# dwkim606/optimal_conv

Measured on AMD Instinct MI355X. Metric: homomorphic convs/sec (conv_then_pack + BN bias, k x k, batch B, N=2^16), higher is better.
Workload: dtype u64; 1 GPU; conv 3 3; ker_wid=3, batch=256, in_wid=16, logN=16, moduli=ckks.DefaultBootstrapParams[6] Q0,Q1 + P=0x1fffffffffe00001, ciphertexts_per_launch_set=4, contexts_per_gpu=4, chunk_nodes=512

## Files before the change

### optimal_conv_amd/csrc/hc_kernels.h

```cpp
#pragma once
#include "hc_arith.h"

#define HC_TPB 256
#ifndef HC_MIN_WAVES
#define HC_MIN_WAVES 4
#endif
#define HC_ROWS_LDS 4096
#define HC_COLS_LDS 4096

struct __attribute__((aligned(16))) HcTw { u64 w, ws; };

#define HC_SMALL_Q(q) ((q) < (1ull << 31))
template <bool B> struct HcBool { static constexpr bool value = B; };
template <int V> struct HcInt { static constexpr int value = V; };
#define HC_COUNT_DISPATCH(n, body) do { switch (n) { case 1: body(HcInt<1>{}); break; case 2: body(HcInt<2>{}); break; case 3: body(HcInt<3>{}); break; case 4: body(HcInt<4>{}); break; \
    case 5: body(HcInt<5>{}); break; case 6: body(HcInt<6>{}); break; case 7: body(HcInt<7>{}); break; case 8: body(HcInt<8>{}); break; default: break; } } while (0)
#define HC_LD(S32, rowptr, j) ((S32) ? hc_ld32(rowptr, j) : (rowptr)[j])
#define HC_ST(S32, rowptr, j, v) do { if (S32) hc_st32(rowptr, j, v); else (rowptr)[j] = (v); } while (0)
#define HC_ROW_DISPATCH(row32, body) do { if (row32) body(HcBool<true>{}); else body(HcBool<false>{}); } while (0)
__device__ __forceinline__ u64 hc_ld32(const u64 *row, size_t j) { return (u64)reinterpret_cast<const u32 *>(row)[j]; }
__device__ __forceinline__ void hc_st32(u64 *row, size_t j, u64 v) { reinterpret_cast<u32 *>(row)[j] = (u32)v; }
struct __attribute__((packed, aligned(4))) HcU64A4 { u64 v; };
__device__ __forceinline__ u64 hc_ldp(const u64 *row, size_t j, bool row32) {
    return reinterpret_cast<const HcU64A4 *>(reinterpret_cast<const char *>(row) + (j << (row32 ? 2 : 3)))->v & (row32 ? 0xFFFFFFFFull : ~0ull);
// ... 146 lines not shown
    hc_gs_round<false>(e, HcRowsTwA<KC>{T.rowsA + row * 16}, Q, T.ninv, T.ninv);
}
template <int FM, bool KC = false>
__device__ __forceinline__ void hc_cols_fwd(u64 (&e)[16], u64 *lds, const HcTwTab &T, int c, int tid, const HcQ &Q) {
    hc_ct_round<FM>(e, HcRowsTwA<KC>{T.colsA}, Q);
#pragma unroll
    for (int hi = 0; hi < 16; hi++) lds[hc_cols_lds(hi * 16 + tid, c)] = e[hi];
    __syncthreads();
#pragma unroll
    for (int lo = 0; lo < 16; lo++) e[lo] = lds[hc_cols_lds(tid * 16 + lo, c)];
    hc_ct_round<FM>(e, HcRowsTwB<KC>{T.colsB + tid}, Q);
}
template <bool SCALE = true, bool KC = false>
__device__ __forceinline__ void hc_cols_inv(u64 (&e)[16], u64 *lds, const HcTwTab &T, int c, int tid, const HcQ &Q) {
    hc_gs_round<false>(e, HcRowsTwB<KC>{T.colsB + tid}, Q, T.ninv, T.ninv);
#pragma unroll
    for (int lo = 0; lo < 16; lo++) lds[hc_cols_lds(tid * 16 + lo, c)] = e[lo];
    __syncthreads();
#pragma unroll
    for (int hi = 0; hi < 16; hi++) e[hi] = lds[hc_cols_lds(hi * 16 + tid, c)];
    hc_gs_round<SCALE>(e, HcRowsTwA<KC>{T.colsA}, Q, T.ninv, T.w_last_ninv);
}

__device__ __forceinline__ void hc_rows_inv_f64(double (&e)[16], u64 *lds, const HcTwTab &T, int row, int rloc, int tid, HcF64Mod m) {
    hc_gs_round_f64<false>(e, HcRowsTwB<false>{T.rowsB + row * 256 + tid}, m, T.ninv, T.ninv);
#pragma unroll
    for (int lo = 0; lo < 16; lo++) lds[hc_rows_lds(rloc, tid * 16 + lo)] = hc_d2u(e[lo]);
    HC_ROW_SYNC();
#pragma unroll
    for (int hi = 0; hi < 16; hi++) e[hi] = hc_u2d(lds[hc_rows_lds(rloc, hi * 16 + tid)]);
    hc_gs_round_f64<false>(e, HcRowsTwA<false>{T.rowsA + row * 16}, m, T.ninv, T.ninv);
}
__device__ __forceinline__ void hc_cols_inv_f64(double (&e)[16], u64 *lds, const HcTwTab &T, int c, int tid, HcF64Mod m) {
    hc_gs_round_f64<false>(e, HcRowsTwB<false>{T.colsB + tid}, m, T.ninv, T.ninv);
#pragma unroll
    for (int lo = 0; lo < 16; lo++) lds[hc_cols_lds(tid * 16 + lo, c)] = hc_d2u(e[lo]);
    __syncthreads();
#pragma unroll
    for (int hi = 0; hi < 16; hi++) e[hi] = hc_u2d(lds[hc_cols_lds(hi * 16 + tid, c)]);
    hc_gs_round_f64<true>(e, HcRowsTwA<false>{T.colsA}, m, T.ninv, T.w_last_ninv);
}

__device__ __forceinline__ void hc_rows_lin_to_lo(u64 (&e)[16], u64 *lds, int t, int rloc, int tid) {
#pragma unroll
    for (int k = 0; k < 16; k++) lds[hc_rows_lds(k, t)] = e[k];
    __syncthreads();
#pragma unroll
    for (int lo = 0; lo < 16; lo++) e[lo] = lds[hc_rows_lds(rloc, tid * 16 + lo)];
}
__device__ __forceinline__ void hc_rows_lo_to_lin(u64 (&e)[16], u64 *lds, int t, int rloc, int tid) {
#pragma unroll
    for (int lo = 0; lo < 16; lo++) lds[hc_rows_lds(rloc, tid * 16 + lo)] = e[lo];
    __syncthreads();
#pragma unroll
    for (int k = 0; k < 16; k++) e[k] = lds[hc_rows_lds(k, t)];
// ... 443 lines not shown
__global__ __launch_bounds__(HC_TPB) void hc_k_permute_mm(const u64 *in, u64 *out, u32 g, size_t is, const HcMod *mods, int nl, int nq, int nt) {
    const size_t base = (size_t)blockIdx.z * is + (size_t)blockIdx.y * 65536;
    const int T = (int)blockIdx.y % nt; const bool row32 = mods[T < nl ? T : nq + (T - nl)].row32 != 0;
    auto body = [&](auto s32c) {
    constexpr bool S32 = decltype(s32c)::value;
    for (size_t i = (size_t)blockIdx.x * HC_TPB + threadIdx.x; i < 65536; i += (size_t)gridDim.x * HC_TPB) HC_ST(S32, out + base, i, HC_LD(S32, in + base, hc_perm_src((u32)i, g)));
    };
    HC_ROW_DISPATCH(row32, body);
}

__global__ __launch_bounds__(HC_TPB) void hc_k_rotate_finish(const u64 *d0, const u64 *d1, const u64 *c0, u64 *o0, u64 *o1, const HcMod *mods, u32 g, size_t is) {
    const int l = blockIdx.y; const u64 q = mods[l].q; const size_t base = (size_t)l * 65536 + (size_t)(blockIdx.z >> 1) * is;
    auto body = [&](auto s32c) {
    constexpr bool S32 = decltype(s32c)::value;
    if ((blockIdx.z & 1) == 0) {
        for (size_t i = (size_t)blockIdx.x * HC_TPB + threadIdx.x; i < 65536; i += (size_t)gridDim.x * HC_TPB) { const size_t s = hc_perm_src((u32)i, g); HC_ST(S32, o0 + base, i, hc_addmod(HC_LD(S32, d0 + base, s), HC_LD(S32, c0 + base, s), q)); }
    } else {
        for (size_t i = (size_t)blockIdx.x * HC_TPB + threadIdx.x; i < 65536; i += (size_t)gridDim.x * HC_TPB) HC_ST(S32, o1 + base, i, HC_LD(S32, d1 + base, hc_perm_src((u32)i, g)));
    }
    };
    HC_ROW_DISPATCH(mods[l].row32, body);
}

#ifndef HC_JOB_FAST
#define HC_JOB_FAST 0
#endif
#if HC_JOB_FAST
#define HC_JOB blockIdx.x
#define HC_TILE blockIdx.y
#define HC_NJOBS gridDim.x
#else
#define HC_JOB blockIdx.y
#define HC_TILE blockIdx.x
#define HC_NJOBS gridDim.y
#endif
#define HC_FREE_OFF 72
#ifndef HC_W_A1
#define HC_W_A1 4
#endif
#ifndef HC_W_A2
#define HC_W_A2 4
#endif
#ifndef HC_W_A3
#define HC_W_A3 4
#endif
#ifndef HC_W_B1
#define HC_W_B1 4
#endif
#ifndef HC_W_B2
#define HC_W_B2 1
#endif
#ifndef HC_W_B3
#define HC_W_B3 4
#endif
#ifndef HC_W_B4
#define HC_W_B4 1
#endif
struct HcLoopA {
    const HcTw *ctc;
    HcPtrs ker;
    u64 *tmp;
    u64 *cts;
    int i0, norm;
    int slot0, slot_step;
    size_t cts_stride;
    int njobs;
    HcMod m0, m1;
    HcTw q1inv;
    u64 h, negh0;
};
#ifndef HC_A_WAVES
#define HC_A_WAVES 4
#endif
template <int F64>
__global__ __launch_bounds__(HC_TPB, HC_W_A1) void hc_k_a1(HcLoopA A, HcTwTab T1inv) {
    __shared__ hc_cvr_lds_t lds[HC_ROWS_LDS];
    const int t = threadIdx.x, tid = t & 15, rloc = t >> 4, row = HC_TILE * 16 + rloc;
    const int job = HC_JOB, p = job & 1, i = A.i0 + (job >> 1) * A.norm, z = blockIdx.z;
    const HcTw *__restrict__ c = A.ctc + ((size_t)z * 4 + (size_t)p * 2 + 1) * 65536;
    const u64 *__restrict__ k = A.ker.p[z] + ((size_t)i * 2 + 1) * 65536;
    const HcQ Q = hc_q(A.m1.q);
    u64 e[16];
#pragma unroll
    for (int kk = 0; kk < 16; kk++) {
        const size_t off = (size_t)(HC_TILE * 16 + kk) * 256 + t;
        const HcTw cw = c[off];
        e[kk] = hc_shoup4(k[off], cw.w, cw.ws, Q);
    }
    u64 *o = A.tmp + ((size_t)z * A.njobs + job) * 65536 + (size_t)row * 256;
    hc_rows_lin_to_lo(e, lds, t, rloc, tid);
    HC_ROW_SYNC();
    if (F64) {
        const HcF64Mod m{(double)A.m1.q, 1.0 / (double)A.m1.q};
        double f[16];
#pragma unroll
        for (int kk = 0; kk < 16; kk++) f[kk] = hc_f64_reduce(hc_f64_from_u(e[kk]), m.q, m.qinv);
        hc_rows_inv_f64(f, lds, T1inv, row, rloc, tid, m);
#pragma unroll
        for (int hi = 0; hi < 16; hi++) o[hi * 16 + tid] = hc_d2u(f[hi]);
    } else {
        hc_rows_inv(e, lds, T1inv, row, rloc, tid, Q);
#pragma unroll
        for (int hi = 0; hi < 16; hi++) o[hi * 16 + tid] = e[hi];
    }
}
template <int FM, int F64>
__global__ __launch_bounds__(HC_TPB, HC_W_A2) void hc_k_a2(HcLoopA A, HcTwTab T1inv, HcTwTab T0fwd) {
    __shared__ hc_cvc_lds_t lds[HC_COLS_LDS];
    const int t = threadIdx.x, c = t & 15, tid = t >> 4;
    u64 *base = A.tmp + (size_t)HC_JOB * 65536 + HC_TILE * 16 + c;
    const HcQ Q0 = hc_q(A.m0.q);
    u64 e[16];
#pragma unroll
    for (int lo = 0; lo < 16; lo++) e[lo] = base[(size_t)(tid * 16 + lo) * 256];
    if (F64) {
        const double q1 = (double)A.m1.q, hh = (double)A.h;
        const HcF64Mod m{q1, 1.0 / q1};
        double f[16];
#pragma unroll
        for (int lo = 0; lo < 16; lo++) f[lo] = hc_u2d(e[lo]);
        hc_cols_inv_f64(f, lds, T1inv, c, tid, m);
#pragma unroll
        for (int hi = 0; hi < 16; hi++) {
            double v = f[hi];
            v = v > hh ? v - q1 : (v < -hh ? v + q1 : v);
            e[hi] = hc_f64_to_u_plus(v, A.m0.q);
        }
    } else {
        const HcQ Q1 = hc_q(A.m1.q);
        hc_cols_inv(e, lds, T1inv, c, tid, Q1);
#pragma unroll
        for (int hi = 0; hi < 16; hi++) {
            const u64 v = hc_csub(hc_canon4(e[hi], Q1) + A.h, A.m1.q);
            e[hi] = hc_reduce64(v + A.negh0, A.m0.mu, Q0);
        }
    }
    __syncthreads();
    hc_cols_fwd<FM>(e, lds, T0fwd, c, tid, Q0);
#pragma unroll
    for (int lo = 0; lo < 16; lo++) base[(size_t)(tid * 16 + lo) * 256] = e[lo];
}
template <int FM>
__global__ __launch_bounds__(HC_TPB, HC_W_A3) void hc_k_a3(HcLoopA A, HcTwTab T0fwd) {
    __shared__ hc_cvr_lds_t lds[HC_ROWS_LDS];
    const int t = threadIdx.x, tid = t & 15, rloc = t >> 4, row = HC_TILE * 16 + rloc;
    const int job = HC_JOB, p = job & 1, i = A.i0 + (job >> 1) * A.norm, z = blockIdx.z;
    const u64 *__restrict__ in = A.tmp + ((size_t)z * A.njobs + job) * 65536 + (size_t)row * 256;
    const HcTw *__restrict__ c = A.ctc + ((size_t)z * 4 + (size_t)p * 2) * 65536 + (size_t)HC_TILE * 4096 + t;
    const u64 *__restrict__ k = A.ker.p[z] + ((size_t)i * 2) * 65536 + (size_t)HC_TILE * 4096 + t;
    u64 *__restrict__ o = A.cts + (size_t)z * A.cts_stride + ((size_t)(A.slot0 + (job >> 1) * A.slot_step) * 2 + p) * 65536 + (size_t)HC_TILE * 4096 + t;
    const HcQ Q = hc_q(A.m0.q);
    u64 e[16], a0[16];
#pragma unroll
    for (int hi = 0; hi < 16; hi++) e[hi] = in[hi * 16 + tid];
#pragma unroll
    for (int kk = 0; kk < 16; kk++) a0[kk] = k[kk * 256];
#pragma unroll
    for (int kk = 0; kk < 16; kk++) { const HcTw cw = c[kk * 256]; a0[kk] = hc_shoup4(a0[kk], cw.w, cw.ws, Q); }
    hc_rows_fwd<FM>(e, lds, T0fwd, row, rloc, tid, Q);
    HC_ROW_SYNC();
    hc_rows_lo_to_lin(e, lds, t, rloc, tid);
#pragma unroll
    for (int kk = 0; kk < 16; kk++) {
        const u64 d = FM == HC_FM_FREE ? a0[kk] + HC_FREE_OFF * Q.q - e[kk] : a0[kk] + Q.q - hc_canon8(e[kk], Q);
        o[kk * 256] = hc_canon4(hc_shoup4(d, A.q1inv.w, A.q1inv.ws, Q), Q);
    }
}

struct HcLoopB {
    const u64 *src;
    u64 *dst;
    u64 *tmpC;
    u64 *tmpE;
    u64 *tmpT;
    const HcTw *idx;
    const HcTw *evkQ;
    const HcTw *evkP;
    const u64 *idxM;
    const u64 *evkQM;
    int n0, step, norm;
    int nodes;
    size_t src_stride, dst_stride;
    HcMod m0, mp;
    HcTw pmodq;
    HcTw pinv;
    u64 mu0;
    u64 vthresh;
    u32 gal;
// ... 25 lines not shown
    hc_rows_inv(e, lds, T0inv, row, rloc, tid, Q);
    u64 *__restrict__ o = B.tmpC + (size_t)job * 65536 + (size_t)row * 256;
#pragma unroll
    for (int hi = 0; hi < 16; hi++) o[hi * 16 + tid] = e[hi];
}
template <int FMP>
__global__ __launch_bounds__(HC_TPB, HC_W_B2) void hc_k_b2(HcLoopB B, HcTwTab T0inv, HcTwTab TPfwd) {
    __shared__ hc_cvc_lds_t lds[HC_COLS_LDS];
    const int t = threadIdx.x, c = t & 15, tid = t >> 4;
    u64 *base = B.tmpC + (size_t)HC_JOB * 65536 + HC_TILE * 16 + c;
    const HcQ Q0 = hc_q(B.m0.q), QP = hc_q(B.mp.q);
    u64 e[16];
#pragma unroll
    for (int lo = 0; lo < 16; lo++) e[lo] = base[(size_t)(tid * 16 + lo) * 256];
    hc_cols_inv(e, lds, T0inv, c, tid, Q0);
#pragma unroll
    for (int hi = 0; hi < 16; hi++) e[hi] = hc_canon4(e[hi], Q0);
    __syncthreads();
    hc_cols_fwd<FMP>(e, lds, TPfwd, c, tid, QP);
#pragma unroll
    for (int lo = 0; lo < 16; lo++) base[(size_t)(tid * 16 + lo) * 256] = e[lo];
}
template <int FMP>
__global__ __launch_bounds__(HC_TPB, HC_W_B3) void hc_k_b3(HcLoopB B, HcTwTab TPfwd, HcTwTab TPinv) {
    __shared__ hc_cvr_lds_t lds[HC_ROWS_LDS];
    const int t = threadIdx.x, tid = t & 15, rloc = t >> 4, row = HC_TILE * 16 + rloc;
    const int node = HC_JOB;
    const u64 *in = B.tmpC + (size_t)node * 65536 + (size_t)row * 256;
    const HcQ Q = hc_q(B.mp.q);
    u64 cp[16], e[16];
#pragma unroll
    for (int hi = 0; hi < 16; hi++) cp[hi] = in[hi * 16 + tid];
    hc_rows_fwd<FMP>(cp, lds, TPfwd, row, rloc, tid, Q);
#pragma unroll
    for (int k = 0; k < 2; k++) {
        const HcTw *__restrict__ ev = B.evkP + (size_t)k * 65536 + (size_t)HC_TILE * 4096 + t;
#pragma unroll
        for (int lo = 0; lo < 16; lo++) {
            const HcTw w = ev[lo * 256];
            e[lo] = hc_shoup4(cp[lo], w.w, w.ws, Q);
        }
        HC_ROW_SYNC();
        hc_rows_inv(e, lds, TPinv, row, rloc, tid, Q);
        u64 *o = B.tmpE + ((size_t)node * 2 + k) * 65536 + (size_t)row * 256;
#pragma unroll
        for (int hi = 0; hi < 16; hi++) o[hi * 16 + tid] = e[hi];
    }
}
template <int FM>
__global__ __launch_bounds__(HC_TPB, HC_W_B4) void hc_k_b4(HcLoopB B, HcTwTab TPinv, HcTwTab T0fwd) {
    __shared__ hc_cvc_lds_t lds[HC_COLS_LDS];
    const int t = threadIdx.x, c = t & 15, tid = t >> 4;
    u64 *base = B.tmpE + (size_t)HC_JOB * 65536 + HC_TILE * 16 + c;
    const HcQ QP = hc_q(B.mp.q), Q = hc_q(B.m0.q);
    u64 e[16];
#pragma unroll
    for (int lo = 0; lo < 16; lo++) e[lo] = base[(size_t)(tid * 16 + lo) * 256];
    hc_cols_inv<false>(e, lds, TPinv, c, tid, QP);
#pragma unroll
    for (int hi = 0; hi < 16; hi++) {
        const u64 yv = hc_canon4(e[hi], QP);
        u64 r = hc_shoup4(yv, B.pinv.w, B.pinv.ws, Q);
        if (yv >= B.vthresh) r += Q.q - 1;
        e[hi] = r;
    }
    __syncthreads();
    hc_cols_fwd<FM>(e, lds, T0fwd, c, tid, Q);
#pragma unroll
    for (int lo = 0; lo < 16; lo++) base[(size_t)(tid * 16 + lo) * 256] = e[lo];
}
// ... 52 lines not shown
                u64 f;
                if (k == 0) hc_b5_terms<FM, 1>(Y[j], T[j], K[j], X[j], I[j], Q, t1[kk], f);
                else hc_b5_terms<FM, 0>(Y[j], T[j], K[j], X[j], I[j], Q, t1[kk], f);
                if (bias != nullptr) t1[kk] = FM == HC_FM_FREE ? t1[kk] + bias[kk * 256] : hc_addmod(t1[kk], bias[kk * 256], q);
                lds[hc_rows_lds(kk, t)] = FM == HC_FM_FREE ? f + HC_FREE_OFF * q - e[kk] : hc_submod(f, hc_canon8(e[kk], Q), q);
            }
        }
        __syncthreads();
#pragma unroll
        for (int kk = 0; kk < 16; kk++) {
            const u32 srcidx = hc_perm_src((u32)((HC_TILE * 16 + kk) * 256 + t), B.gal);
            const u64 d = lds[hc_rows_lds((int)((srcidx >> 8) & 15), (int)(srcidx & 255))];
            o[kk * 256] = FM == HC_FM_FREE ? hc_reduce64(t1[kk] + d, B.m0.mu, Q) : hc_addmod(t1[kk], d, q);
        }
    }
}

#ifndef HC_B5_ROWS
#define HC_B5_ROWS 4
#endif
#ifndef HC_B5M_WAVES
#define HC_B5M_WAVES 2
#endif
template <int FM, class TW>
__device__ __forceinline__ void hc_ct_round2(u64 (&e0)[16], u64 (&e1)[16], const TW &tw, const HcQ &Q) {
#pragma unroll
    for (int s = 0; s < 4; s++) {
        const int half = 8 >> s;
#pragma unroll
        for (int g = 0; g < (1 << s); g++) {
            const HcTw w = tw((1 << s) - 1 + g);
#pragma unroll
            for (int k = 0; k < half; k++) {
                const int a = g * 2 * half + k, b = a + half;
                u64 X0 = e0[a], X1 = e1[a];
                if (FM == HC_FM_ALT) { X0 = hc_fold(X0, Q.nq4); X1 = hc_fold(X1, Q.nq4); }
                const u64 T0 = hc_shoup4(e0[b], w.w, w.ws, Q), T1 = hc_shoup4(e1[b], w.w, w.ws, Q);
                e0[a] = X0 + T0; e0[b] = (X0 + Q.q4) - T0;
                e1[a] = X1 + T1; e1[b] = (X1 + Q.q4) - T1;
            }
        }
    }
}
template <int FM>
__device__ __forceinline__ void hc_rows_fwd2_lin(u64 (&e0)[16], u64 (&e1)[16], u64 *l0, u64 *l1, const HcTwTab &T, int row, int rloc, int tid, int t, const HcQ &Q) {
    hc_ct_round2<FM>(e0, e1, HcRowsTwA<false>{T.rowsA + row * 16}, Q);
#pragma unroll
    for (int hi = 0; hi < 16; hi++) { const int a = hc_rows_lds(rloc, hi * 16 + tid); l0[a] = e0[hi]; l1[a] = e1[hi]; }
    HC_ROW_SYNC();
#pragma unroll
    for (int lo = 0; lo < 16; lo++) { const int a = hc_rows_lds(rloc, tid * 16 + lo); e0[lo] = l0[a]; e1[lo] = l1[a]; }
    hc_ct_round2<FM>(e0, e1, HcRowsTwB<false>{T.rowsB + row * 256 + tid}, Q);
    HC_ROW_SYNC();
#pragma unroll
    for (int lo = 0; lo < 16; lo++) { const int a = hc_rows_lds(rloc, tid * 16 + lo); l0[a] = e0[lo]; l1[a] = e1[lo]; }
    __syncthreads();
#pragma unroll
    for (int k = 0; k < 16; k++) { const int a = hc_rows_lds(k, t); e0[k] = l0[a]; e1[k] = l1[a]; }
}
template <int FM>
__global__ __launch_bounds__(HC_TPB, HC_B5M_WAVES) void hc_k_b5m(HcLoopB B, HcTwTab T0fwd, HcPtrs biases, HcPtrs outs) {
    __shared__ u64 lds[2 * HC_ROWS_LDS];
    u64 *l0 = lds, *l1 = lds + HC_ROWS_LDS;
    const int t = threadIdx.x, tid = t & 15, rloc = t >> 4, row = HC_TILE * 16 + rloc;
    const int zn = HC_JOB, z = zn / B.nodes, node = zn - z * B.nodes, i = (B.n0 + node) * B.norm;
    const HcQ Q = hc_q(B.m0.q);
// ... 1436 lines not shown
```

### optimal_conv_amd/csrc/hconv.hip

```cpp
#ifdef HC_EMU
#include "hip_emu.h"
#else
#include <hip/hip_runtime.h>
#endif

#include <math.h>
#include <stdarg.h>
#include <stdio.h>
#include <string.h>

#include <map>
#include <utility>
#include <string>
#include <vector>

#include "../../include/hconv.h"
#include "../../include/hconv_test_hooks.h"
#include "hc_kernels.h"
#include "hc_gomath.h"
#ifndef HC_GX_LV
#define HC_GX_LV 64
#endif
#ifndef HC_GX_PW
#define HC_GX_PW 32
// ... 667 lines not shown
    c->ws_ctc = nullptr; c->ws_ctc_cts = 0;
    HC_HIP(c, hcx_malloc(c, (void **)&c->ws_ctc, nct * 4 * HC_N * sizeof(HcTw)));
    c->ws_ctc_cts = nct;
    return HC_OK;
}
static int hc_prepare_ctc(hc_ctx *c, const HcPtrs &ct_in, int n, const u64 cst[2]) {
    HC_TRY(hc_ensure_ctc(c, (size_t)n));
    HcCtc K; K.m0 = c->mods[0].m; K.m1 = c->mods[1].m;
    K.c0 = h_pair(cst[0] % K.m0.q, K.m0.q); K.c1 = h_pair(cst[1] % K.m1.q, K.m1.q);
    return hc_launch(c, "ctc", hc_k_ctc_pairs, dim3(64, 4, (unsigned)n), ct_in, c->ws_ctc, K);
}

static int hc_loopA_run_set(hc_ctx *c, const HcPtrs &kers, int n, int i_first, int i_stride, int nch, u64 *cts, size_t cts_stride, bool compact) {
    long chunk = (c->chunk_nodes < 1 ? 1 : c->chunk_nodes) / n; if (chunk < 1) chunk = 1;
    if (chunk > nch) chunk = nch;
    HC_TRY(hc_ensure_tmp(c, (size_t)n * (size_t)chunk * 2));
    HcLoopA A; HC_TRY(hc_fill_loopA(c, &A, kers, cts, cts_stride, i_stride));
    const HcModHost &m0 = c->mods[0], &m1 = c->mods[1];
    for (int j0 = 0; j0 < nch; j0 += (int)chunk) {
        const int nj = (int)((nch - j0) < chunk ? (nch - j0) : chunk);
        A.i0 = i_first + j0 * i_stride;
        A.slot0 = compact ? j0 : A.i0; A.slot_step = compact ? 1 : i_stride;
        A.njobs = 2 * nj;
        const dim3 grid = hc_grid(2 * nj, n), flat = hc_grid(2 * nj * n);
        if (hc_f64_ok(m1.m.q)) {
            HC_TRY(hc_launch(c, "a1_mul_rowsinv", hc_k_a1<1>, grid, A, m1.inv_f64));
            HC_TRY(hc_fm_free(m0.m.q) ? hc_launch(c, "a2_colsinv_lift_colsfwd", hc_k_a2<HC_FM_FREE, 1>, flat, A, m1.inv_f64, m0.fwd)
                                      : hc_launch(c, "a2_colsinv_lift_colsfwd", hc_k_a2<HC_FM_ALT, 1>, flat, A, m1.inv_f64, m0.fwd));
        } else {
            HC_TRY(hc_launch(c, "a1_mul_rowsinv", hc_k_a1<0>, grid, A, m1.inv));
            HC_TRY(hc_fm_free(m0.m.q) ? hc_launch(c, "a2_colsinv_lift_colsfwd", hc_k_a2<HC_FM_FREE, 0>, flat, A, m1.inv, m0.fwd)
                                      : hc_launch(c, "a2_colsinv_lift_colsfwd", hc_k_a2<HC_FM_ALT, 0>, flat, A, m1.inv, m0.fwd));
        }
        HC_TRY(HC_LAUNCH_FM(m0.m.q, c, "a3_rowsfwd_rescale", hc_k_a3, grid, A, m0.fwd));
    }
    return HC_OK;
}
static int hc_loopA_run(hc_ctx *c, const u64 *ker, int max_ob, int norm, u64 *cts) {
    return hc_loopA_run_set(c, hc_ptrs1(ker), 1, 0, norm, max_ob / norm, cts, 0, false);
}

static int hc_rescale_plan(hc_ctx *c, int level, const HcTw **out) {
    auto it = c->rescale_plan.find(level);
    if (it == c->rescale_plan.end()) {
        const u64 qL = c->mods[(size_t)level].m.q;
        std::vector<HcTw> h((size_t)level);
        for (int i = 0; i < level; i++) { const u64 q = c->mods[(size_t)i].m.q; h[(size_t)i] = h_pair(h_inv(qL % q, q), q); }
        HcTw *d = nullptr; HC_HIP(c, hcx_malloc(c, (void **)&d, h.size() * sizeof(HcTw)));
        HC_HIP(c, hcx_h2d(c, d, h.data(), h.size() * sizeof(HcTw)));
        it = c->rescale_plan.emplace(level, d).first;
    }
    *out = it->second;
    return HC_OK;
}
static int hc_div_round_last_n(hc_ctx *c, int level, const u64 *x, size_t xs, u64 *out, size_t os, int np) {
    if (level < 1 || level >= c->nq) return hc_fail(c, HC_ERR_ARG, "hc_div_round_last: level %d outside 1..%d", level, c->nq - 1);
    if (!x || !out) return hc_fail(c, HC_ERR_ARG, "hc_div_round_last: null");
// ... 227 lines not shown
    HC_TRY(hc_ensure_tmp(c, (size_t)n * chunk * 4));
    HcLoopB B; HC_TRY(hc_fill_loopB(c, &B, src, dst, it->second, logStep, step, norm, galEl, n * chunk));
    B.src_stride = sstride; B.dst_stride = dstride;
    if (it->second.row256) B.tmpT = nullptr;
    HcPtrs nobias; memset(&nobias, 0, sizeof nobias);
    const HcModHost &m0 = c->mods[0], &mp = c->mods[(size_t)c->nq];
    for (int n0 = 0; n0 < nodes; n0 += chunk) {
        const int nn = (nodes - n0) < chunk ? (nodes - n0) : chunk;
        B.n0 = n0; B.nodes = nn;
        const dim3 g1 = hc_grid(n * nn), g2 = hc_grid(2 * n * nn);
        if (c->small_levels > 0 && (long)n * nn <= c->small_levels && it->second.row256 && !HC_JOB_FAST) {
            const HcPtrs pb = bias_last ? *bias_last : nobias, po = outs_last ? *outs_last : nobias;
            B.tmpT = nullptr;
            const dim3 s1(HC_STILES, (unsigned)(n * nn)), s2(HC_STILES, (unsigned)(2 * n * nn)), s3(HC_STILES, (unsigned)(n * nn), 2);
            HC_TRY(hc_launch<HC_STPB>(c, "b1_node_rowsinv", hc_k_sb1, s1, B, m0.inv));
            HC_TRY(hc_launch<HC_STPB>(c, "b2_colsinv_colsfwdP", hc_k_sb2, s1, B, m0.inv, mp.fwd));
            HC_TRY(hc_launch<HC_STPB>(c, "b3_rowsfwdP_mac_rowsinvP", hc_k_sb3, s3, B, mp.fwd, mp.inv));
            HC_TRY(hc_launch<HC_STPB>(c, "b4_colsinvP_modup_colsfwd", hc_k_sb4, s2, B, mp.inv, m0.fwd));
            HC_TRY(hc_launch<HC_STPB>(c, "b5_rowsfwd_moddown_perm_add", hc_k_sb5, s2, B, m0.fwd, pb, po));
            continue;
        }
        HC_TRY(hc_launch(c, "b1_node_rowsinv", hc_k_b1, g1, B, m0.inv));
        HC_TRY(HC_LAUNCH_FM(mp.m.q, c, "b2_colsinv_colsfwdP", hc_k_b2, g1, B, m0.inv, mp.fwd));
        HC_TRY(HC_LAUNCH_FM(mp.m.q, c, "b3_rowsfwdP_mac_rowsinvP", hc_k_b3, g1, B, mp.fwd, mp.inv));
        HC_TRY(HC_LAUNCH_FM(m0.m.q, c, "b4_colsinvP_modup_colsfwd", hc_k_b4, g2, B, mp.inv, m0.fwd));
        const HcPtrs pb = bias_last ? *bias_last : nobias, po = outs_last ? *outs_last : nobias;
        if (it->second.row256) HC_TRY(HC_LAUNCH_FM(m0.m.q, c, "b5_rowsfwd_moddown_perm_add", hc_k_b5m, g1, B, m0.fwd, pb, po));
        else HC_TRY(HC_LAUNCH_FM(m0.m.q, c, "b5_rowsfwd_moddown_perm_add", hc_k_b5, g2, B, m0.fwd, pb, po));
    }
    return HC_OK;
}
static int hc_pack_run(hc_ctx *c, u64 *cts, size_t cstride, int n, int max_cnum, int real_cnum, const HcPtrs *bias, int stride_log2 = 0, const HcPtrs *outs = nullptr) {
    if (max_cnum < 1 || real_cnum < 1 || max_cnum % real_cnum || (max_cnum & (max_cnum - 1)) || (real_cnum & (real_cnum - 1)))
        return hc_fail(c, HC_ERR_ARG, "pack: max_cnum=%d real_cnum=%d must be powers of two", max_cnum, real_cnum);
    const int norm = max_cnum / real_cnum;
    int step = max_cnum / 2, logStep = 0;
    for (int i = step; i > 1; i /= 2) logStep++;
    if (stride_log2 < 0 || logStep + stride_log2 >= HC_LOGN) return hc_fail(c, HC_ERR_ARG, "pack: stride_log2=%d out of range", stride_log2);
    int j = HC_LOGN - logStep - stride_log2;
    const size_t pong_one = (size_t)(max_cnum / 2 > 0 ? max_cnum / 2 : 1) * 2, pong_rows = pong_one * (size_t)n;
    if (c->ws_cts2_rows < pong_rows) {
        HC_HIP(c, hipStreamSynchronize(c->stream));
        if (c->ws_cts2) HC_HIP(c, hcx_free(c, c->ws_cts2));
        c->ws_cts2 = nullptr; c->ws_cts2_rows = 0;
        HC_HIP(c, hcx_malloc(c, (void **)&c->ws_cts2, pong_rows * HC_N * sizeof(u64)));
        c->ws_cts2_rows = pong_rows;
    }
// ... 30 lines not shown
}

extern "C" int hc_rotate_gal_l0(hc_ctx *c, uint64_t galEl, const uint64_t *c0, const uint64_t *c1, uint64_t *o0, uint64_t *o1);
static int hc_ks_common(hc_ctx *c, uint64_t galEl, const uint64_t *c0, const uint64_t *c1, uint64_t *o0, uint64_t *o1, bool rotate) {
    auto it = c->evk.find(galEl);
    if (it == c->evk.end()) return hc_fail(c, HC_ERR_STATE, "no switching key loaded for galEl=%llu", (unsigned long long)galEl);
    u64 *buf = nullptr; HC_HIP(c, hcx_malloc(c, (void **)&buf, (size_t)6 * HC_N * sizeof(u64)));
    u64 *y = buf, *x = buf + 2 * HC_N, *res = buf + 4 * HC_N;
    int rc = HC_OK;
    hipError_t he = hipMemsetAsync(x, 0, 2 * HC_N * sizeof(u64), c->stream);
    if (he == hipSuccess) he = c0 ? hipMemcpyAsync(y, c0, HC_N * sizeof(u64), hipMemcpyDeviceToDevice, c->stream) : hipMemsetAsync(y, 0, HC_N * sizeof(u64), c->stream);
    if (he == hipSuccess) he = hipMemcpyAsync(y + HC_N, c1, HC_N * sizeof(u64), hipMemcpyDeviceToDevice, c->stream);
    if (he != hipSuccess) rc = hc_fail(c, HC_ERR_HIP, "level-0 key switch: staging copies failed: %s", hipGetErrorString(he));
    if (!rc && !c->idx_pairs) rc = hc_idx_load(c, nullptr);
    const bool local = it->second.row_local;
    if (!rc) {
        if (rotate && local) {
            const int chunk = 1;
            rc = hc_ensure_tmp(c, 4);
            HcLoopB B; if (!rc) rc = hc_fill_loopB(c, &B, y, res, it->second, 0, 1, 1, galEl, chunk);
            const HcModHost &m0 = c->mods[0], &mp = c->mods[(size_t)c->nq];
            if (!rc) rc = hc_launch(c, "b1_node_rowsinv", hc_k_b1, hc_grid(1), B, m0.inv);
            if (!rc) rc = HC_LAUNCH_FM(mp.m.q, c, "b2_colsinv_colsfwdP", hc_k_b2, hc_grid(1), B, m0.inv, mp.fwd);
            if (!rc) rc = HC_LAUNCH_FM(mp.m.q, c, "b3_rowsfwdP_mac_rowsinvP", hc_k_b3, hc_grid(1), B, mp.fwd, mp.inv);
            if (!rc) rc = HC_LAUNCH_FM(m0.m.q, c, "b4_colsinvP_modup_colsfwd", hc_k_b4, hc_grid(2), B, mp.inv, m0.fwd);
            HcPtrs nobias; memset(&nobias, 0, sizeof nobias);
            if (!rc) rc = HC_LAUNCH_FM(m0.m.q, c, "b5_rowsfwd_moddown_perm_add", hc_k_b5, hc_grid(2), B, m0.fwd, nobias, nobias);
            HcTw z; z.w = z.ws = 0;
            if (!rc) rc = hc_launch(c, "ks_sub", hc_k_pointwise<HC_PW_SUB>, hc_pw_grid(2 * HC_N), (const u64 *)res, (const u64 *)y, res, (size_t)2 * HC_N, c->mods[0].m, z);
            if (!rc && (hipMemcpyAsync(o0, res, HC_N * sizeof(u64), hipMemcpyDeviceToDevice, c->stream) != hipSuccess
                        || hipMemcpyAsync(o1, res + HC_N, HC_N * sizeof(u64), hipMemcpyDeviceToDevice, c->stream) != hipSuccess)) rc = hc_fail(c, HC_ERR_HIP, "level-0 key switch: result copies failed");
        } else {
            rc = hc_fail(c, HC_ERR_UNSUPPORTED, "level-0 key switch is exposed for Galois elements that permute inside 4096-coefficient tiles (2^j+1, j>=5), the ones pack_ctxts uses");
        }
    }
    if (hipStreamSynchronize(c->stream) != hipSuccess && !rc) rc = hc_fail(c, HC_ERR_HIP, "level-0 key switch: stream synchronize failed");
    if (hcx_free(c, buf) != hipSuccess && !rc) rc = hc_fail(c, HC_ERR_HIP, "level-0 key switch: free failed");
    return rc;
}
extern "C" int hc_rotate_gal_l0(hc_ctx *c, uint64_t galEl, const uint64_t *c0, const uint64_t *c1, uint64_t *o0, uint64_t *o1) {
    HC_ENTER(c); if (!c0 || !c1 || !o0 || !o1) return hc_fail(c, HC_ERR_ARG, "hc_rotate_gal_l0: null");
    return hc_ks_common(c, galEl, c0, c1, o0, o1, true);
}
extern "C" int hc_keyswitch_l0(hc_ctx *c, uint64_t galEl, const uint64_t *c1, uint64_t *d0, uint64_t *d1) {
    HC_ENTER(c); if (!c1 || !d0 || !d1) return hc_fail(c, HC_ERR_ARG, "hc_keyswitch_l0: null");
    u64 *buf = nullptr; HC_HIP(c, hcx_malloc(c, (void **)&buf, (size_t)2 * HC_N * sizeof(u64)));
    int rc = hc_ks_common(c, galEl, nullptr, c1, buf, buf + HC_N, true);
// ... 655 lines not shown
```

Baseline: 785.4 conv/s.

## Process both ciphertext halves per block in a1, a3 and b3 NTT kernels

The a1 and a3 kernels now handle the p=0 and p=1 ciphertext components in a single block, so the kernel coefficient row is loaded once and the twiddle loads and LDS exchanges are shared across two NTTs, with half as many blocks launched. The b3 kernel likewise computes both key-switch products in one pass with a paired inverse NTT instead of looping over them. Paired NTT and GS round helpers were added to support this, and the minimum waves for a1 and a3 drop from 4 to 3 to allow for the higher register use. The cost is more register pressure and extra barriers in the paired LDS exchange, and fewer blocks means less parallelism.

```diff
diff --git a/optimal_conv_amd/csrc/hc_kernels.h b/optimal_conv_amd/csrc/hc_kernels.h
--- a/optimal_conv_amd/csrc/hc_kernels.h
+++ b/optimal_conv_amd/csrc/hc_kernels.h
@@ -192,15 +192,6 @@
     hc_gs_round<SCALE>(e, HcRowsTwA<KC>{T.colsA}, Q, T.ninv, T.w_last_ninv);
 }
 
-__device__ __forceinline__ void hc_rows_inv_f64(double (&e)[16], u64 *lds, const HcTwTab &T, int row, int rloc, int tid, HcF64Mod m) {
-    hc_gs_round_f64<false>(e, HcRowsTwB<false>{T.rowsB + row * 256 + tid}, m, T.ninv, T.ninv);
-#pragma unroll
-    for (int lo = 0; lo < 16; lo++) lds[hc_rows_lds(rloc, tid * 16 + lo)] = hc_d2u(e[lo]);
-    HC_ROW_SYNC();
-#pragma unroll
-    for (int hi = 0; hi < 16; hi++) e[hi] = hc_u2d(lds[hc_rows_lds(rloc, hi * 16 + tid)]);
-    hc_gs_round_f64<false>(e, HcRowsTwA<false>{T.rowsA + row * 16}, m, T.ninv, T.ninv);
-}
 __device__ __forceinline__ void hc_cols_inv_f64(double (&e)[16], u64 *lds, const HcTwTab &T, int c, int tid, HcF64Mod m) {
     hc_gs_round_f64<false>(e, HcRowsTwB<false>{T.colsB + tid}, m, T.ninv, T.ninv);
 #pragma unroll
@@ -690,6 +681,99 @@
     HC_ROW_DISPATCH(mods[l].row32, body);
 }
 
+template <int FM, class TW>
+__device__ __forceinline__ void hc_ct_round2(u64 (&e0)[16], u64 (&e1)[16], const TW &tw, const HcQ &Q) {
+#pragma unroll
+    for (int s = 0; s < 4; s++) {
+        const int half = 8 >> s;
+#pragma unroll
+        for (int g = 0; g < (1 << s); g++) {
+            const HcTw w = tw((1 << s) - 1 + g);
+#pragma unroll
+            for (int k = 0; k < half; k++) {
+                const int a = g * 2 * half + k, b = a + half;
+                u64 X0 = e0[a], X1 = e1[a];
+                if (FM == HC_FM_ALT) { X0 = hc_fold(X0, Q.nq4); X1 = hc_fold(X1, Q.nq4); }
+                const u64 T0 = hc_shoup4(e0[b], w.w, w.ws, Q), T1 = hc_shoup4(e1[b], w.w, w.ws, Q);
+                e0[a] = X0 + T0; e0[b] = (X0 + Q.q4) - T0;
+                e1[a] = X1 + T1; e1[b] = (X1 + Q.q4) - T1;
+            }
+        }
+    }
+}
+template <class TW>
+__device__ __forceinline__ void hc_gs_round2(u64 (&e0)[16], u64 (&e1)[16], const TW &tw, const HcQ &Q) {
+#pragma unroll
+    for (int s = 0; s < 4; s++) {
+        const int dist = 1 << s;
+#pragma unroll
+        for (int g = 0; g < (8 >> s); g++) {
+            const HcTw w = tw((8 >> s) - 1 + g);
+#pragma unroll
+            for (int k = 0; k < dist; k++) {
+                const int a = g * 2 * dist + k, b = a + dist;
+                const u64 X0 = e0[a], Y0 = e0[b], X1 = e1[a], Y1 = e1[b];
+                e0[a] = hc_fold(X0 + Y0, Q.nq4); e0[b] = hc_shoup4((X0 + Q.q4) - Y0, w.w, w.ws, Q);
+                e1[a] = hc_fold(X1 + Y1, Q.nq4); e1[b] = hc_shoup4((X1 + Q.q4) - Y1, w.w, w.ws, Q);
+            }
+        }
+    }
+}
+template <class TW>
+__device__ __forceinline__ void hc_gs_round2_f64(double (&e0)[16], double (&e1)[16], const TW &tw, HcF64Mod m) {
+#pragma unroll
+    for (int s = 0; s < 4; s++) {
+        const int dist = 1 << s;
+#pragma unroll
+        for (int g = 0; g < (8 >> s); g++) {
+            const HcTw w = tw((8 >> s) - 1 + g);
+            const double ww = hc_u2d(w.w), wq = hc_u2d(w.ws);
+#pragma unroll
+            for (int k = 0; k < dist; k++) {
+                const int a = g * 2 * dist + k, b = a + dist;
+                const double X0 = e0[a], Y0 = e0[b], X1 = e1[a], Y1 = e1[b], u0 = X0 + Y0, u1 = X1 + Y1;
+                e0[a] = (s & 1) ? hc_f64_reduce(u0, m.q, m.qinv) : u0; e0[b] = hc_f64_mulmod(X0 - Y0, ww, wq, m.q);
+                e1[a] = (s & 1) ? hc_f64_reduce(u1, m.q, m.qinv) : u1; e1[b] = hc_f64_mulmod(X1 - Y1, ww, wq, m.q);
+            }
+        }
+    }
+}
+template <class WA, class RA, class SY>
+__device__ __forceinline__ void hc_xchg2(u64 (&e0)[16], u64 (&e1)[16], u64 *lds, WA wa, RA ra, SY sync) {
+#pragma unroll
+    for (int i = 0; i < 16; i++) lds[wa(i)] = e0[i];
+    sync();
+#pragma unroll
+    for (int i = 0; i < 16; i++) e0[i] = lds[ra(i)];
+    sync();
+#pragma unroll
+    for (int i = 0; i < 16; i++) lds[wa(i)] = e1[i];
+    sync();
+#pragma unroll
+    for (int i = 0; i < 16; i++) e1[i] = lds[ra(i)];
+}
+template <int FM>
+__device__ __forceinline__ void hc_rows_fwd2(u64 (&e0)[16], u64 (&e1)[16], u64 *lds, const HcTwTab &T, int row, int rloc, int tid, const HcQ &Q) {
+    hc_ct_round2<FM>(e0, e1, HcRowsTwA<false>{T.rowsA + row * 16}, Q);
+    hc_xchg2(e0, e1, lds, [&](int hi) { return hc_rows_lds(rloc, hi * 16 + tid); }, [&](int lo) { return hc_rows_lds(rloc, tid * 16 + lo); }, [] { HC_ROW_SYNC(); });
+    hc_ct_round2<FM>(e0, e1, HcRowsTwB<false>{T.rowsB + row * 256 + tid}, Q);
+}
+__device__ __forceinline__ void hc_rows_inv2(u64 (&e0)[16], u64 (&e1)[16], u64 *lds, const HcTwTab &T, int row, int rloc, int tid, const HcQ &Q) {
+    hc_gs_round2(e0, e1, HcRowsTwB<false>{T.rowsB + row * 256 + tid}, Q);
+    hc_xchg2(e0, e1, lds, [&](int lo) { return hc_rows_lds(rloc, tid * 16 + lo); }, [&](int hi) { return hc_rows_lds(rloc, hi * 16 + tid); }, [] { HC_ROW_SYNC(); });
+    hc_gs_round2(e0, e1, HcRowsTwA<false>{T.rowsA + row * 16}, Q);
+}
+__device__ __forceinline__ void hc_rows_inv2_f64(double (&f0)[16], double (&f1)[16], u64 *lds, const HcTwTab &T, int row, int rloc, int tid, HcF64Mod m) {
+    hc_gs_round2_f64(f0, f1, HcRowsTwB<false>{T.rowsB + row * 256 + tid}, m);
+    u64 b0[16], b1[16];
+#pragma unroll
+    for (int i = 0; i < 16; i++) { b0[i] = hc_d2u(f0[i]); b1[i] = hc_d2u(f1[i]); }
+    hc_xchg2(b0, b1, lds, [&](int lo) { return hc_rows_lds(rloc, tid * 16 + lo); }, [&](int hi) { return hc_rows_lds(rloc, hi * 16 + tid); }, [] { HC_ROW_SYNC(); });
+#pragma unroll
+    for (int i = 0; i < 16; i++) { f0[i] = hc_u2d(b0[i]); f1[i] = hc_u2d(b1[i]); }
+    hc_gs_round2_f64(f0, f1, HcRowsTwA<false>{T.rowsA + row * 16}, m);
+}
+
 #ifndef HC_JOB_FAST
 #define HC_JOB_FAST 0
 #endif
@@ -704,13 +788,13 @@
 #endif
 #define HC_FREE_OFF 72
 #ifndef HC_W_A1
-#define HC_W_A1 4
+#define HC_W_A1 3
 #endif
 #ifndef HC_W_A2
 #define HC_W_A2 4
 #endif
 #ifndef HC_W_A3
-#define HC_W_A3 4
+#define HC_W_A3 3
 #endif
 #ifndef HC_W_B1
 #define HC_W_B1 4
@@ -723,6 +807,9 @@
 #endif
 #ifndef HC_W_B4
 #define HC_W_B4 1
+#endif
+#ifndef HC_A3_ROWS
+#define HC_A3_ROWS 4
 #endif
 struct HcLoopA {
     const HcTw *ctc;
@@ -737,39 +824,37 @@
     HcTw q1inv;
     u64 h, negh0;
 };
-#ifndef HC_A_WAVES
-#define HC_A_WAVES 4
-#endif
 template <int F64>
-__global__ __launch_bounds__(HC_TPB, HC_W_A1) void hc_k_a1(HcLoopA A, HcTwTab T1inv) {
+__global__ __launch_bounds__(HC_TPB, HC_W_A1) void hc_k_a1p(HcLoopA A, HcTwTab T1inv) {
     __shared__ hc_cvr_lds_t lds[HC_ROWS_LDS];
     const int t = threadIdx.x, tid = t & 15, rloc = t >> 4, row = HC_TILE * 16 + rloc;
-    const int job = HC_JOB, p = job & 1, i = A.i0 + (job >> 1) * A.norm, z = blockIdx.z;
-    const HcTw *__restrict__ c = A.ctc + ((size_t)z * 4 + (size_t)p * 2 + 1) * 65536;
-    const u64 *__restrict__ k = A.ker.p[z] + ((size_t)i * 2 + 1) * 65536;
+    const int ch = HC_JOB, i = A.i0 + ch * A.norm, z = blockIdx.z;
+    const HcTw *__restrict__ c0 = A.ctc + ((size_t)z * 4 + 1) * 65536 + (size_t)HC_TILE * 4096 + t;
+    const u64 *__restrict__ k = A.ker.p[z] + ((size_t)i * 2 + 1) * 65536 + (size_t)HC_TILE * 4096 + t;
     const HcQ Q = hc_q(A.m1.q);
-    u64 e[16];
+    u64 e0[16], e1[16];
 #pragma unroll
     for (int kk = 0; kk < 16; kk++) {
-        const size_t off = (size_t)(HC_TILE * 16 + kk) * 256 + t;
-        const HcTw cw = c[off];
-        e[kk] = hc_shoup4(k[off], cw.w, cw.ws, Q);
-    }
-    u64 *o = A.tmp + ((size_t)z * A.njobs + job) * 65536 + (size_t)row * 256;
-    hc_rows_lin_to_lo(e, lds, t, rloc, tid);
+        const u64 kv = k[kk * 256];
+        const HcTw w0 = c0[kk * 256], w1 = c0[2 * 65536 + kk * 256];
+        e0[kk] = hc_shoup4(kv, w0.w, w0.ws, Q);
+        e1[kk] = hc_shoup4(kv, w1.w, w1.ws, Q);
+    }
+    u64 *o = A.tmp + ((size_t)z * A.njobs + 2 * ch) * 65536 + (size_t)row * 256;
+    hc_xchg2(e0, e1, lds, [&](int kk) { return hc_rows_lds(kk, t); }, [&](int lo) { return hc_rows_lds(rloc, tid * 16 + lo); }, [] { __syncthreads(); });
     HC_ROW_SYNC();
     if (F64) {
         const HcF64Mod m{(double)A.m1.q, 1.0 / (double)A.m1.q};
-        double f[16];
-#pragma unroll
-        for (int kk = 0; kk < 16; kk++) f[kk] = hc_f64_reduce(hc_f64_from_u(e[kk]), m.q, m.qinv);
-        hc_rows_inv_f64(f, lds, T1inv, row, rloc, tid, m);
-#pragma unroll
-        for (int hi = 0; hi < 16; hi++) o[hi * 16 + tid] = hc_d2u(f[hi]);
+        double f0[16], f1[16];
+#pragma unroll
+        for (int kk = 0; kk < 16; kk++) { f0[kk] = hc_f64_reduce(hc_f64_from_u(e0[kk]), m.q, m.qinv); f1[kk] = hc_f64_reduce(hc_f64_from_u(e1[kk]), m.q, m.qinv); }
+        hc_rows_inv2_f64(f0, f1, lds, T1inv, row, rloc, tid, m);
+#pragma unroll
+        for (int hi = 0; hi < 16; hi++) { o[hi * 16 + tid] = hc_d2u(f0[hi]); o[65536 + hi * 16 + tid] = hc_d2u(f1[hi]); }
     } else {
-        hc_rows_inv(e, lds, T1inv, row, rloc, tid, Q);
-#pragma unroll
-        for (int hi = 0; hi < 16; hi++) o[hi * 16 + tid] = e[hi];
+        hc_rows_inv2(e0, e1, lds, T1inv, row, rloc, tid, Q);
+#pragma unroll
+        for (int hi = 0; hi < 16; hi++) { o[hi * 16 + tid] = e0[hi]; o[65536 + hi * 16 + tid] = e1[hi]; }
     }
 }
 template <int FM, int F64>
@@ -809,29 +894,37 @@
     for (int lo = 0; lo < 16; lo++) base[(size_t)(tid * 16 + lo) * 256] = e[lo];
 }
 template <int FM>
-__global__ __launch_bounds__(HC_TPB, HC_W_A3) void hc_k_a3(HcLoopA A, HcTwTab T0fwd) {
+__global__ __launch_bounds__(HC_TPB, HC_W_A3) void hc_k_a3p(HcLoopA A, HcTwTab T0fwd) {
     __shared__ hc_cvr_lds_t lds[HC_ROWS_LDS];
     const int t = threadIdx.x, tid = t & 15, rloc = t >> 4, row = HC_TILE * 16 + rloc;
-    const int job = HC_JOB, p = job & 1, i = A.i0 + (job >> 1) * A.norm, z = blockIdx.z;
-    const u64 *__restrict__ in = A.tmp + ((size_t)z * A.njobs + job) * 65536 + (size_t)row * 256;
-    const HcTw *__restrict__ c = A.ctc + ((size_t)z * 4 + (size_t)p * 2) * 65536 + (size_t)HC_TILE * 4096 + t;
+    const int ch = HC_JOB, i = A.i0 + ch * A.norm, z = blockIdx.z;
+    const u64 *__restrict__ in = A.tmp + ((size_t)z * A.njobs + 2 * ch) * 65536 + (size_t)row * 256;
+    const HcTw *__restrict__ c0 = A.ctc + (size_t)z * 4 * 65536 + (size_t)HC_TILE * 4096 + t;
     const u64 *__restrict__ k = A.ker.p[z] + ((size_t)i * 2) * 65536 + (size_t)HC_TILE * 4096 + t;
-    u64 *__restrict__ o = A.cts + (size_t)z * A.cts_stride + ((size_t)(A.slot0 + (job >> 1) * A.slot_step) * 2 + p) * 65536 + (size_t)HC_TILE * 4096 + t;
+    u64 *__restrict__ o = A.cts + (size_t)z * A.cts_stride + (size_t)(A.slot0 + ch * A.slot_step) * 2 * 65536 + (size_t)HC_TILE * 4096 + t;
     const HcQ Q = hc_q(A.m0.q);
-    u64 e[16], a0[16];
-#pragma unroll
-    for (int hi = 0; hi < 16; hi++) e[hi] = in[hi * 16 + tid];
-#pragma unroll
-    for (int kk = 0; kk < 16; kk++) a0[kk] = k[kk * 256];
-#pragma unroll
-    for (int kk = 0; kk < 16; kk++) { const HcTw cw = c[kk * 256]; a0[kk] = hc_shoup4(a0[kk], cw.w, cw.ws, Q); }
-    hc_rows_fwd<FM>(e, lds, T0fwd, row, rloc, tid, Q);
+    u64 e0[16], e1[16], kv[16];
+#pragma unroll
+    for (int hi = 0; hi < 16; hi++) { e0[hi] = in[hi * 16 + tid]; e1[hi] = in[65536 + hi * 16 + tid]; }
+#pragma unroll
+    for (int kk = 0; kk < 16; kk++) kv[kk] = k[kk * 256];
+    hc_rows_fwd2<FM>(e0, e1, lds, T0fwd, row, rloc, tid, Q);
     HC_ROW_SYNC();
-    hc_rows_lo_to_lin(e, lds, t, rloc, tid);
-#pragma unroll
-    for (int kk = 0; kk < 16; kk++) {
-        const u64 d = FM == HC_FM_FREE ? a0[kk] + HC_FREE_OFF * Q.q - e[kk] : a0[kk] + Q.q - hc_canon8(e[kk], Q);
-        o[kk * 256] = hc_canon4(hc_shoup4(d, A.q1inv.w, A.q1inv.ws, Q), Q);
+    hc_xchg2(e0, e1, lds, [&](int lo) { return hc_rows_lds(rloc, tid * 16 + lo); }, [&](int kk) { return hc_rows_lds(kk, t); }, [] { __syncthreads(); });
+#pragma unroll
+    for (int b = 0; b < 16; b += HC_A3_ROWS) {
+        HcTw w0[HC_A3_ROWS], w1[HC_A3_ROWS];
+#pragma unroll
+        for (int j = 0; j < HC_A3_ROWS; j++) { w0[j] = c0[(b + j) * 256]; w1[j] = c0[2 * 65536 + (b + j) * 256]; }
+#pragma unroll
+        for (int j = 0; j < HC_A3_ROWS; j++) {
+            const int kk = b + j;
+            const u64 a0 = hc_shoup4(kv[kk], w0[j].w, w0[j].ws, Q), a1 = hc_shoup4(kv[kk], w1[j].w, w1[j].ws, Q);
+            const u64 d0 = FM == HC_FM_FREE ? a0 + HC_FREE_OFF * Q.q - e0[kk] : a0 + Q.q - hc_canon8(e0[kk], Q);
+            const u64 d1 = FM == HC_FM_FREE ? a1 + HC_FREE_OFF * Q.q - e1[kk] : a1 + Q.q - hc_canon8(e1[kk], Q);
+            o[kk * 256] = hc_canon4(hc_shoup4(d0, A.q1inv.w, A.q1inv.ws, Q), Q);
+            o[65536 + kk * 256] = hc_canon4(hc_shoup4(d1, A.q1inv.w, A.q1inv.ws, Q), Q);
+        }
     }
 }
 
@@ -903,30 +996,31 @@
     for (int lo = 0; lo < 16; lo++) base[(size_t)(tid * 16 + lo) * 256] = e[lo];
 }
 template <int FMP>
-__global__ __launch_bounds__(HC_TPB, HC_W_B3) void hc_k_b3(HcLoopB B, HcTwTab TPfwd, HcTwTab TPinv) {
+__global__ __launch_bounds__(HC_TPB, HC_W_B3) void hc_k_b3p(HcLoopB B, HcTwTab TPfwd, HcTwTab TPinv) {
     __shared__ hc_cvr_lds_t lds[HC_ROWS_LDS];
     const int t = threadIdx.x, tid = t & 15, rloc = t >> 4, row = HC_TILE * 16 + rloc;
     const int node = HC_JOB;
     const u64 *in = B.tmpC + (size_t)node * 65536 + (size_t)row * 256;
     const HcQ Q = hc_q(B.mp.q);
-    u64 cp[16], e[16];
-#pragma unroll
-    for (int hi = 0; hi < 16; hi++) cp[hi] = in[hi * 16 + tid];
-    hc_rows_fwd<FMP>(cp, lds, TPfwd, row, rloc, tid, Q);
-#pragma unroll
-    for (int k = 0; k < 2; k++) {
-        const HcTw *__restrict__ ev = B.evkP + (size_t)k * 65536 + (size_t)HC_TILE * 4096 + t;
+    u64 e0[16], e1[16];
+    {
+        u64 cp[16];
+#pragma unroll
+        for (int hi = 0; hi < 16; hi++) cp[hi] = in[hi * 16 + tid];
+        hc_rows_fwd<FMP>(cp, lds, TPfwd, row, rloc, tid, Q);
+        const HcTw *__restrict__ ev = B.evkP + (size_t)HC_TILE * 4096 + t;
 #pragma unroll
         for (int lo = 0; lo < 16; lo++) {
-            const HcTw w = ev[lo * 256];
-            e[lo] = hc_shoup4(cp[lo], w.w, w.ws, Q);
-        }
-        HC_ROW_SYNC();
-        hc_rows_inv(e, lds, TPinv, row, rloc, tid, Q);
-        u64 *o = B.tmpE + ((size_t)node * 2 + k) * 65536 + (size_t)row * 256;
-#pragma unroll
-        for (int hi = 0; hi < 16; hi++) o[hi * 16 + tid] = e[hi];
-    }
+            const HcTw w0 = ev[lo * 256], w1 = ev[65536 + lo * 256];
+            e0[lo] = hc_shoup4(cp[lo], w0.w, w0.ws, Q);
+            e1[lo] = hc_shoup4(cp[lo], w1.w, w1.ws, Q);
+        }
+    }
+    HC_ROW_SYNC();
+    hc_rows_inv2(e0, e1, lds, TPinv, row, rloc, tid, Q);
+    u64 *o = B.tmpE + (size_t)node * 2 * 65536 + (size_t)row * 256;
+#pragma unroll
+    for (int hi = 0; hi < 16; hi++) { o[hi * 16 + tid] = e0[hi]; o[65536 + hi * 16 + tid] = e1[hi]; }
 }
 template <int FM>
 __global__ __launch_bounds__(HC_TPB, HC_W_B4) void hc_k_b4(HcLoopB B, HcTwTab TPinv, HcTwTab T0fwd) {
@@ -1025,26 +1119,6 @@
 #ifndef HC_B5M_WAVES
 #define HC_B5M_WAVES 2
 #endif
-template <int FM, class TW>
-__device__ __forceinline__ void hc_ct_round2(u64 (&e0)[16], u64 (&e1)[16], const TW &tw, const HcQ &Q) {
-#pragma unroll
-    for (int s = 0; s < 4; s++) {
-        const int half = 8 >> s;
-#pragma unroll
-        for (int g = 0; g < (1 << s); g++) {
-            const HcTw w = tw((1 << s) - 1 + g);
-#pragma unroll
-            for (int k = 0; k < half; k++) {
-                const int a = g * 2 * half + k, b = a + half;
-                u64 X0 = e0[a], X1 = e1[a];
-                if (FM == HC_FM_ALT) { X0 = hc_fold(X0, Q.nq4); X1 = hc_fold(X1, Q.nq4); }
-                const u64 T0 = hc_shoup4(e0[b], w.w, w.ws, Q), T1 = hc_shoup4(e1[b], w.w, w.ws, Q);
-                e0[a] = X0 + T0; e0[b] = (X0 + Q.q4) - T0;
-                e1[a] = X1 + T1; e1[b] = (X1 + Q.q4) - T1;
-            }
-        }
-    }
-}
 template <int FM>
 __device__ __forceinline__ void hc_rows_fwd2_lin(u64 (&e0)[16], u64 (&e1)[16], u64 *l0, u64 *l1, const HcTwTab &T, int row, int rloc, int tid, int t, const HcQ &Q) {
     hc_ct_round2<FM>(e0, e1, HcRowsTwA<false>{T.rowsA + row * 16}, Q);
diff --git a/optimal_conv_amd/csrc/hconv.hip b/optimal_conv_amd/csrc/hconv.hip
--- a/optimal_conv_amd/csrc/hconv.hip
+++ b/optimal_conv_amd/csrc/hconv.hip
@@ -713,17 +713,17 @@
         A.i0 = i_first + j0 * i_stride;
         A.slot0 = compact ? j0 : A.i0; A.slot_step = compact ? 1 : i_stride;
         A.njobs = 2 * nj;
-        const dim3 grid = hc_grid(2 * nj, n), flat = hc_grid(2 * nj * n);
+        const dim3 pair = hc_grid(nj, n), flat = hc_grid(2 * nj * n);
         if (hc_f64_ok(m1.m.q)) {
-            HC_TRY(hc_launch(c, "a1_mul_rowsinv", hc_k_a1<1>, grid, A, m1.inv_f64));
+            HC_TRY(hc_launch(c, "a1_mul_rowsinv", hc_k_a1p<1>, pair, A, m1.inv_f64));
             HC_TRY(hc_fm_free(m0.m.q) ? hc_launch(c, "a2_colsinv_lift_colsfwd", hc_k_a2<HC_FM_FREE, 1>, flat, A, m1.inv_f64, m0.fwd)
                                       : hc_launch(c, "a2_colsinv_lift_colsfwd", hc_k_a2<HC_FM_ALT, 1>, flat, A, m1.inv_f64, m0.fwd));
         } else {
-            HC_TRY(hc_launch(c, "a1_mul_rowsinv", hc_k_a1<0>, grid, A, m1.inv));
+            HC_TRY(hc_launch(c, "a1_mul_rowsinv", hc_k_a1p<0>, pair, A, m1.inv));
             HC_TRY(hc_fm_free(m0.m.q) ? hc_launch(c, "a2_colsinv_lift_colsfwd", hc_k_a2<HC_FM_FREE, 0>, flat, A, m1.inv, m0.fwd)
                                       : hc_launch(c, "a2_colsinv_lift_colsfwd", hc_k_a2<HC_FM_ALT, 0>, flat, A, m1.inv, m0.fwd));
         }
-        HC_TRY(HC_LAUNCH_FM(m0.m.q, c, "a3_rowsfwd_rescale", hc_k_a3, grid, A, m0.fwd));
+        HC_TRY(HC_LAUNCH_FM(m0.m.q, c, "a3_rowsfwd_rescale", hc_k_a3p, pair, A, m0.fwd));
     }
     return HC_OK;
 }
@@ -997,7 +997,7 @@
         }
         HC_TRY(hc_launch(c, "b1_node_rowsinv", hc_k_b1, g1, B, m0.inv));
         HC_TRY(HC_LAUNCH_FM(mp.m.q, c, "b2_colsinv_colsfwdP", hc_k_b2, g1, B, m0.inv, mp.fwd));
-        HC_TRY(HC_LAUNCH_FM(mp.m.q, c, "b3_rowsfwdP_mac_rowsinvP", hc_k_b3, g1, B, mp.fwd, mp.inv));
+        HC_TRY(HC_LAUNCH_FM(mp.m.q, c, "b3_rowsfwdP_mac_rowsinvP", hc_k_b3p, g1, B, mp.fwd, mp.inv));
         HC_TRY(HC_LAUNCH_FM(m0.m.q, c, "b4_colsinvP_modup_colsfwd", hc_k_b4, g2, B, mp.inv, m0.fwd));
         const HcPtrs pb = bias_last ? *bias_last : nobias, po = outs_last ? *outs_last : nobias;
         if (it->second.row256) HC_TRY(HC_LAUNCH_FM(m0.m.q, c, "b5_rowsfwd_moddown_perm_add", hc_k_b5m, g1, B, m0.fwd, pb, po));
@@ -1074,7 +1074,7 @@
             const HcModHost &m0 = c->mods[0], &mp = c->mods[(size_t)c->nq];
             if (!rc) rc = hc_launch(c, "b1_node_rowsinv", hc_k_b1, hc_grid(1), B, m0.inv);
             if (!rc) rc = HC_LAUNCH_FM(mp.m.q, c, "b2_colsinv_colsfwdP", hc_k_b2, hc_grid(1), B, m0.inv, mp.fwd);
-            if (!rc) rc = HC_LAUNCH_FM(mp.m.q, c, "b3_rowsfwdP_mac_rowsinvP", hc_k_b3, hc_grid(1), B, mp.fwd, mp.inv);
+            if (!rc) rc = HC_LAUNCH_FM(mp.m.q, c, "b3_rowsfwdP_mac_rowsinvP", hc_k_b3p, hc_grid(1), B, mp.fwd, mp.inv);
             if (!rc) rc = HC_LAUNCH_FM(m0.m.q, c, "b4_colsinvP_modup_colsfwd", hc_k_b4, hc_grid(2), B, mp.inv, m0.fwd);
             HcPtrs nobias; memset(&nobias, 0, sizeof nobias);
             if (!rc) rc = HC_LAUNCH_FM(m0.m.q, c, "b5_rowsfwd_moddown_perm_add", hc_k_b5, hc_grid(2), B, m0.fwd, nobias, nobias);
```

Measured after the change: 813.3 conv/s (median of 6 runs). 3.5% higher.
